# RegulatoryGenomicsGroup/chicdiff

Measured on AMD Instinct MI355X. Metric: interactions/sec NB-GLM Wald test, higher is better.
Workload: dtype f64; 1 GPU; synthetic 2000000 interactions x 8 samples (4v4), size factors + offsets(theta=0.5) + dispersions + Wald, design ~condition; rows_per_gpu=2000000, samples=8, global_rows=2000000, parallelism=rows-sharded x1, collectives=none (single rank), ranks_in_communicator=1

## Files before the change

### chicdiff_amd/csrc/api.hip

```cpp
#include <math.h>
#include <stdarg.h>
#include <stdio.h>
#include <stdlib.h>
#include <string.h>

#include <algorithm>
#include <mutex>
#include <thread>
#include <string>
#include <vector>
#include <unordered_set>

#include <dlfcn.h>

#include "common.h"
#include "prior_mc.h"

using namespace cd;

namespace cd {
struct ChinputCols {
    std::vector<int32_t> bait, oe, N;
    std::string error;
};
// ... 45 lines not shown
    struct EarlyCopy {
        int n = 0;
        struct Item { int col; char *pin; size_t bytes; } item[10];
        hipEvent_t ready = nullptr, done = nullptr;
        bool issued = false;
    } *early = nullptr;
    hipStream_t copy_stream = nullptr;
    hipEvent_t ev_fork = nullptr, ev_join = nullptr;
    std::vector<chicdiff_hip_ctx *> lanes;
    int cu_count = 0;
    hipStream_t own_stream = nullptr, stream = nullptr;
    chicdiff_allreduce_fn allreduce = nullptr;
    void *allreduce_user = nullptr;
    chicdiff_allgather_fn allgather = nullptr;
    void *allgather_user = nullptr;
    int world = 1, rank = 0;
    void *rccl_lib = nullptr, *rccl_comm = nullptr;
    int (*rccl_allreduce)(const void *, void *, size_t, int, int, void *, hipStream_t) = nullptr;
    int (*rccl_allgather)(const void *, void *, size_t, int, void *, hipStream_t) = nullptr;
    int (*rccl_comm_destroy)(void *) = nullptr;
    const char *(*rccl_error_string)(int) = nullptr;
    char err[512] = {0};
    int64_t cap_n = 0;
    int cap_S = 0;
    void *ws = nullptr;
    size_t ws_bytes = 0;
    char *aux = nullptr;
    size_t aux_bytes = 0;
    FitWork w{};
    double *d_sf = nullptr;
    double *d_logfact = nullptr;
    PmcTable *d_pmc[4] = {nullptr, nullptr, nullptr, nullptr};
    double *d_nf_tmp = nullptr;
    FitScalars *h_sc = nullptr;
    double *h_sf = nullptr;
    int timing = 0;
    std::vector<KTimer> timers;
    std::vector<std::pair<int, hipEvent_t>> pending;
    std::vector<hipEvent_t> event_pool;
    int scope_depth = 0;
    std::unordered_set<void *> user_allocs;
    std::mutex user_mu;
};

static char g_create_err[512];
constexpr int64_t kFuseOffsetsMaxRows = 1 << 18;

static const PmcTable &pmc_table(int df) {
    static PmcTable tables[4];
    static bool ready[4] = {false, false, false, false};
    static std::mutex mu;
    std::lock_guard<std::mutex> lock(mu);
    if (!ready[df]) {
        pmc_build(df, tables[df]);
        ready[df] = true;
    }
    return tables[df];
}

static int fail(chicdiff_hip_ctx *c, int code, const char *fmt, ...) {
    va_list ap;
    va_start(ap, fmt);
    vsnprintf(c ? c->err : g_create_err, 512, fmt, ap);
    va_end(ap);
    return code;
}
// ... 302 lines not shown
extern "C" int32_t chicdiff_hip_kernel_times(chicdiff_hip_ctx *c, chicdiff_kernel_time *out, int32_t cap) {
    if (!c) return 0;
    int32_t k = 0;
    for (auto &t : c->timers) {
        if (t.launches == 0) continue;
        if (out && k < cap) {
            out[k].name = t.name.c_str();
            out[k].ms = t.ms;
            out[k].launches = t.launches;
            out[k].bytes = t.bytes;
        }
        k++;
    }
    return k;
}

static size_t align256(size_t x) { return (x + 255) & ~(size_t)255; }

static int ensure_workspace(chicdiff_hip_ctx *c, int64_t n, int S) {
    if (c->ws && n <= c->cap_n && S <= c->cap_S) return CHICDIFF_OK;
    if (c->ws) {
        HIPCHK(c, hipStreamSynchronize(c->stream));
        HIPCHK(c, hipFree(c->ws));
        c->ws = nullptr;
    }
    const size_t nd = align256(sizeof(double) * (size_t)n), ni = align256(sizeof(int32_t) * (size_t)n);
    const size_t n_double_arrays = 15, n_int_arrays = 9;
    const size_t partials = align256(sizeof(double) * ((size_t)kRedBlocks * 72 + 128));
    const size_t hist = align256(sizeof(double) * (size_t)kMaxS * 2 * kSelBins);
    const size_t nfbytes = align256(sizeof(double) * (size_t)n * S);
    const size_t selcnt = align256(sizeof(double) * (size_t)kSelMaxWorld * kMaxS * 2);
    const size_t rowpack = align256((size_t)row_stride(S) * (size_t)n);
    const size_t start4 = align256(sizeof(double) * 4 * (size_t)n);
    const size_t total = nd * n_double_arrays + ni * n_int_arrays + partials + 2 * hist + selcnt + align256(sizeof(FitScalars)) + kQueueBytes + 1024 + kPlaceWords * 8 + nfbytes + rowpack + start4;
    hipError_t e = hipMalloc(&c->ws, total);
    if (e != hipSuccess) return fail(c, CHICDIFF_E_NOMEM, "workspace of %zu bytes: %s", total, hipGetErrorString(e));
    c->ws_bytes = total;
    char *p = (char *)c->ws;
    auto takeD = [&](double *&ptr) { ptr = (double *)p; p += nd; };
    auto takeI = [&](int32_t *&ptr) { ptr = (int32_t *)p; p += ni; };
    FitWork &w = c->w;
    takeD(w.baseMean); takeD(w.baseVar); takeD(w.gm0); takeD(w.gm1); takeD(w.rough); takeD(w.binit0); takeD(w.binit1);
    takeD(w.crow); takeD(w.dispGene); takeD(w.dispFit); takeD(w.dispMAP); takeD(w.disp); takeD(w.beta0); takeD(w.beta1);
    takeD(w.resid);
    takeI(w.allZero); takeI(w.geneIter); takeI(w.mapIter); takeI(w.outlier); takeI(w.betaIter); takeI(w.optimConv);
    takeI(w.order);
    { int32_t *q; takeI(q); w.cls = (uint8_t *)q; }
    takeI(w.gridlist);
    w.partials = (double *)p; p += partials;
    w.hist = (double *)p; p += hist;
    w.hist_local = (double *)p; p += hist;
    w.selcnt = (double *)p; p += selcnt;
    w.sc = (FitScalars *)p; p += align256(sizeof(FitScalars));
    w.logfact = c->d_logfact;
    w.queue = (unsigned long long *)p; p += kQueueBytes;
    w.barrier = (unsigned int *)p; p += 1024;
    w.place = (unsigned long long *)p; p += kPlaceWords * 8;
    c->d_nf_tmp = (double *)p; p += nfbytes;
    w.rowpack = p; p += rowpack;
    w.start = (double *)p;
    c->cap_n = n;
    c->cap_S = S;
    HIPCHK(c, hipMemsetAsync(w.sc, 0, align256(sizeof(FitScalars)) + kQueueBytes + 1024, c->stream));
    return CHICDIFF_OK;
}

static int ensure_aux(chicdiff_hip_ctx *c, size_t bytes) {
    if (c->aux_bytes >= bytes) return CHICDIFF_OK;
    if (c->aux) {
        HIPCHK(c, hipStreamSynchronize(c->stream));
        HIPCHK(c, hipFree(c->aux));
        c->aux = nullptr;
        c->aux_bytes = 0;
    }
    hipError_t e = hipMalloc((void **)&c->aux, bytes);
    if (e != hipSuccess) return fail(c, CHICDIFF_E_NOMEM, "scratch of %zu bytes: %s", bytes, hipGetErrorString(e));
    c->aux_bytes = bytes;
    return CHICDIFF_OK;
}

struct CollTimer {
    chicdiff_hip_ctx *c;
    int idx = -1;
    hipEvent_t e0 = nullptr, e1 = nullptr;
    CollTimer(chicdiff_hip_ctx *c_, const char *name, double bytes) : c(c_) {
        if (c->timing != 1) return;
        for (size_t i = 0; i < c->timers.size(); i++)
            if (c->timers[i].name == name) idx = (int)i;
        if (idx < 0) {
            KTimer t;
            t.name = name;
            c->timers.push_back(t);
            idx = (int)c->timers.size() - 1;
// ... 747 lines not shown
    auto cleanup = [&]() {
        if (early.issued) (void)hipStreamSynchronize(c->copy_stream);
        if (early.ready) (void)hipEventDestroy(early.ready);
        if (early.done) (void)hipEventDestroy(early.done);
    };
    if (rc) { cleanup(); return rc; }
    for (auto &q : cols) {
        if (q.early) continue;
        if (e == hipSuccess) e = hipEventCreateWithFlags(&q.ev, hipEventDisableTiming);
        if (e == hipSuccess) e = hipMemcpyAsync(q.pin, q.dev, q.bytes, hipMemcpyDeviceToHost, c->stream);
        if (e == hipSuccess) e = hipEventRecord(q.ev, c->stream);
    }
    if (e == hipSuccess && !cols.empty()) {
        std::sort(cols.begin(), cols.end(), [](const Col &x, const Col &y) { return x.early > y.early; });
        int nt = c->host.host_copy_threads < (int)cols.size() ? c->host.host_copy_threads : (int)cols.size();
        std::vector<std::thread> th;
        for (int t = 0; t < nt; t++)
            th.emplace_back([&, t]() {
                for (size_t k = t; k < cols.size(); k += nt) {
                    if (hipEventSynchronize(cols[k].early ? early.done : cols[k].ev) != hipSuccess) { trc[0] = 1; continue; }
                    memcpy(cols[k].host, cols[k].pin, cols[k].bytes);
                }
            });
        for (auto &w : th) w.join();
    }
    for (auto &q : cols) if (q.ev) (void)hipEventDestroy(q.ev);
    cleanup();
    if (e != hipSuccess || trc[0]) return fail(c, CHICDIFF_E_HIP, "D2H copy: %s", e != hipSuccess ? hipGetErrorString(e) : "event wait failed");
    return CHICDIFF_OK;
}

static int size_factors_impl(chicdiff_hip_ctx *c, const int32_t *d_counts, int64_t n, int32_t S, bool all_rounds) {
    Scope t(c, "size_factors");
    launch_row_ratio(d_counts, n, S, c->d_nf_tmp, c->d_carry, c->stream);
    SelArgs sa{};
    sa.mode = SEL_SIZEFACTOR;
    sa.ncol = S;
    sa.n = n;
    sa.ratio = c->d_nf_tmp;
    sa.S = S;
    sa.sf_out = c->d_sf;
    sa.overflow_out = c->d_carry;
    const int rc = run_select(c, sa, all_rounds);
    if (rc) return rc;
    if (c->host.fault_inject & 4) {
        c->host.fault_inject &= ~4;
        launch_poke(c->d_carry, 1, c->stream);
    }
    return CHICDIFF_OK;
}

static int sf_overflow_consensus(chicdiff_hip_ctx *c, bool *overflow) {
    double *d_flag = c->d_sf + kMaxS;
    launch_flag_to_double(c->d_carry, d_flag, c->stream);
    int rc = do_allreduce(c, d_flag, 1);
    if (rc) return rc;
    double h = 0;
    HIPCHK(c, hipMemcpyAsync(&h, d_flag, sizeof h, hipMemcpyDeviceToHost, c->stream));
    HIPCHK(c, hipStreamSynchronize(c->stream));
    *overflow = h > 0;
    return CHICDIFF_OK;
}

int chicdiff_hip_size_factors_dev(chicdiff_hip_ctx *c, const int32_t *d_counts, int64_t n, int32_t S, double *sf_host) {
    if (!c) return CHICDIFF_E_INVALID;
    int rc = (!d_counts || !sf_host || n < 1 || S < 1 || S > kMaxS) ? fail(c, CHICDIFF_E_INVALID, "size_factors: bad arguments") : CHICDIFF_OK;
    if ((rc = begin_call(c, rc, n, S))) return rc;
    bool all_rounds = c->host.select_all_rounds != 0, overflow = false;
    for (;;) {
        if ((rc = size_factors_impl(c, d_counts, n, S, all_rounds)) || (rc = sf_overflow_consensus(c, &overflow))) break;
        if (!overflow || all_rounds) break;
        all_rounds = true;
        c->refits++;
    }
    if (!rc) rc = read_scalars(c);
    timing_collect(c);
    if (rc) return rc;
// ... 220 lines not shown
    if (!d_counts || !d_nf || !d_log_alpha || !d_lp || !d_dlp || !d_alpha || !d_mu || K < 1 || live_rows < 0 || live_rows > 64 ||
        (d_prior_mean && !(prior_var > 0)))
        return fail(c, CHICDIFF_E_INVALID, "selftest_objective: bad arguments");
    if (int rc = check_counts_group(c, n, S, group, d)) return rc;
    if (int rc = check_opts(c, opts)) return rc;
    HIPCHK(c, hipSetDevice(c->device));
    if (int rc = ensure_workspace(c, n, S)) return rc;
    const Opts o = make_opts(c, opts, S);
    HIPCHK(c, hipMemsetAsync(c->w.sc, 0, align256(sizeof(FitScalars)) + kQueueBytes + 1024, c->stream));
    launch_prep(d_counts, const_cast<double *>(d_nf), d, c->w, o, c->stream);
    ObjectiveProbe pb{d_log_alpha, K, d_prior_mean, d_prior_mean ? 1.0 / prior_var : 0.0, live_rows, d_lp, d_dlp, d_alpha, d_mu};
    const int lanes = launch_objective_probe(d, c->w, o, pb, c->stream);
    HIPCHK(c, hipStreamSynchronize(c->stream));
    if (lanes < 0) return fail(c, CHICDIFF_E_INVALID, "selftest_objective: the line search has no samples-across-lanes layout for %d live rows at S = %d", live_rows, S);
    HIPCHK(c, hipGetLastError());
    if (lanes_per_row) *lanes_per_row = lanes;
    return CHICDIFF_OK;
}

extern "C" int chicdiff_hip_selftest_r_random(int32_t kind, uint32_t seed, double a, double b, int64_t n, double *out) {
    if (!out || n < 0 || kind < 0 || kind > 3) return CHICDIFF_E_INVALID;
    if (kind == 3 && !(a > 0 && b > 0)) return CHICDIFF_E_INVALID;
    RStream r(seed);
    for (int64_t i = 0; i < n; i++) out[i] = kind == 0 ? r.unif() : kind == 1 ? r.norm() : kind == 2 ? r.expo() : r.gamma(a, b);
    return CHICDIFF_OK;
}
extern "C" int chicdiff_hip_selftest_sched_class(int32_t mode, double min_disp, const double *alpha_init, const double *group_mean, int64_t n,
                                                 int32_t *cls_out, int32_t *bounds) {
    if (n < 0 || (n > 0 && (!alpha_init || !group_mean || !cls_out)) || mode < 1 || mode > 4) return CHICDIFF_E_INVALID;
    for (int64_t i = 0; i < n; i++) cls_out[i] = cd::sched_class(alpha_init[i], group_mean[i], min_disp, mode);
    if (bounds) for (int a = 0; a <= 6; a++) bounds[a] = cd::sched_classes_a(a, mode);
    return CHICDIFF_OK;
}
extern "C" int chicdiff_hip_selftest_queue_claim(uint64_t old, int32_t back, uint32_t chunks, uint32_t first_back, int32_t stop_percent, int32_t claimed,
                                                 uint32_t *chunk_out, int32_t *again_out) {
    uint32_t chunk = 0;
    const bool valid = cd::queue_claim(old, back != 0, chunks, chunk);
    if (chunk_out) *chunk_out = chunk;
    if (again_out) *again_out = cd::filler_claims(claimed != 0, old, chunks, first_back, cd::filler_stop_f(stop_percent, chunks, first_back));
    return valid ? 1 : 0;
}
extern "C" int chicdiff_hip_selftest_prior_mc(int32_t df, const double *hist40, double *dens_out, double *prior_var_out) {
    if (df < 1 || df > 3) return CHICDIFF_E_INVALID;
    const PmcTable &t = pmc_table(df);
    if (dens_out) memcpy(dens_out, t.dens, sizeof t.dens);
    if (prior_var_out) {
        if (!hist40) return CHICDIFF_E_INVALID;
        *prior_var_out = pmc_prior_var(hist40, t);
    }
    return CHICDIFF_OK;
}

extern "C" int chicdiff_hip_fragment_background_dev(chicdiff_hip_ctx *c, const int32_t *d_bait, const int32_t *d_oe, int64_t nru,
                                                    int32_t id_min, int32_t nid, const int64_t *d_midsum, int32_t S,
                                                    const double *d_sj, const double *d_si, const int32_t *d_tblb,
                                                    const int32_t *d_tlb, const double *d_T, int32_t ntblb, int32_t ntlb,
                                                    const double *distfun_host, double *d_bmean, double *d_tmean,
                                                    double *d_fullmean) {
    if (!c) return CHICDIFF_E_INVALID;
    if (!d_bait || !d_oe || !d_midsum || !d_sj || !d_si || !d_tblb || !d_tlb || !d_T || !distfun_host || nru < 0 || nid < 1 ||
        S < 1 || S > kMaxS || ntblb < 1 || ntlb < 1)
        return fail(c, CHICDIFF_E_INVALID, "fragment_background: bad arguments");
    HIPCHK(c, hipSetDevice(c->device));
    int rc = ensure_aux(c, sizeof(double) * 10 * kMaxS);
    if (rc) return rc;
    double *d_df = reinterpret_cast<double *>(c->aux);
// ... 389 lines not shown
```

### chicdiff_amd/csrc/common.h

```cpp
#pragma once
#include <hip/hip_runtime.h>
#include <stdint.h>

#include "../../include/chicdiff_hip.h"
#include "fit_driver.h"
#include "fit_state.h"

namespace cd {

constexpr int kRedBlocks = 1024;

struct FitDims {
    int64_t n;
    int32_t S, p, nA, nB;
    uint64_t gmask;
};

struct FitWork {
    double *baseMean, *baseVar, *gm0, *gm1, *rough, *binit0, *binit1, *crow;
    double *dispGene, *dispFit, *dispMAP, *disp, *beta0, *beta1, *resid;
    int32_t *allZero, *geneIter, *mapIter, *outlier, *betaIter, *optimConv;
    int32_t *order;
    uint8_t *cls;
    int32_t *gridlist;
// ... 143 lines not shown
void launch_dispfit_resid(FitDims d, FitWork w, Opts o, hipStream_t st);
void launch_prior_var(FitDims d, FitWork w, Opts o, hipStream_t st);
void launch_resid_hist(FitDims d, FitWork w, double *out40, hipStream_t st);
void launch_prior_mc(FitDims d, FitWork w, const double *hist40, const void *table, hipStream_t st);
void launch_wald_prep(const int32_t *counts, const double *nf, FitDims d, FitWork w, Opts o, hipStream_t st);
void launch_wald_irls(const int32_t *counts, const double *nf, FitDims d, FitWork w, Opts o, hipStream_t st);
void launch_wald_final(const int32_t *counts, const double *nf, FitDims d, FitWork w, Opts o,
                       const chicdiff_nbglm_out &out, hipStream_t st);
void launch_wald_intercept(const int32_t *counts, const double *nf, FitDims d, FitWork w, Opts o,
                           const chicdiff_nbglm_out &out, hipStream_t st);
void launch_dev_sum_finish(FitDims d, FitWork w, const int32_t *carry, const double *sf_dev, hipStream_t st);

struct SelArgs {
    int mode;
    int ncol;
    int64_t n;
    const double *resid;
    const double *ratio;
    int S;
    int shift;
    double *sf_out;
    int32_t *overflow_out;
};
void launch_sel_hist(SelArgs a, FitWork w, hipStream_t st);
void launch_sel_step(SelArgs a, FitWork w, hipStream_t st);
void launch_sel_shortcut(SelArgs a, FitWork w, hipStream_t st);
void launch_sel_finish(SelArgs a, FitWork w, hipStream_t st);
void launch_sel_keep_local(SelArgs a, FitWork w, hipStream_t st);
void launch_sel_gather_counts(SelArgs a, FitWork w, int world, int rank, hipStream_t st);
void launch_sel_gather_place(SelArgs a, FitWork w, int world, int rank, hipStream_t st);
void launch_sel_gather_finish(SelArgs a, FitWork w, int world, int rank, hipStream_t st);

void launch_row_ratio(const int32_t *counts, int64_t n, int S, double *ratio, int32_t *clear_flag, hipStream_t st);
void launch_offsets(const double *fullMean, const double *sf_dev, int64_t n, int S, double theta, int mix,
                    double *out, hipStream_t st);
void launch_window_sums(const int32_t *fragN, const double *fragFM, int64_t nfrag, int S, const int64_t *rptr,
                        int64_t n, int32_t *N, double *FM, hipStream_t st);
size_t count_join_scratch_bytes(int64_t nkeys);
void launch_count_join(const int32_t *bait, const int32_t *oe, int64_t nru, const int64_t *keys,
                       const int32_t *vals, int64_t nkeys, int32_t *out, void *scratch, hipStream_t st);
void launch_fragment_background(const int32_t *bait, const int32_t *oe, int64_t nru, int32_t id_min, int32_t nid,
                                const int64_t *midsum, int32_t S, const double *sj, const double *si, const int32_t *tblb,
                                const int32_t *tlb, const double *T, int32_t ntblb, int32_t ntlb, const double *distfun_dev,
                                double *bmean, double *tmean, double *fullmean, hipStream_t st);
size_t bh_workspace_bytes(int64_t n);
int launch_bh_adjust(const double *p, int64_t n, double *padj, char *ws, hipStream_t st);
size_t ihw_workspace_bytes();
void launch_ihw_apply(const double *avDist, const double *pvalue, int64_t n, const double *breaks, const double *weights,
                      int ng, int32_t *group, double *weight, double *wp, double *partials, hipStream_t st);
void launch_cooks_filter(const int32_t *counts, int64_t n, int S, int p, const double *maxCooks, const int32_t *argmax,
                         double cutoff, double *pvalue, unsigned long long *nout, hipStream_t st);
size_t if_workspace_bytes(int64_t n);
int run_independent_filtering(const double *d_bm, const double *d_p, int64_t n, double alpha, double *d_padj, char *ws, hipStream_t st,
                              hipStream_t st2, hipEvent_t fork, hipEvent_t join, chicdiff_results_info *info);
size_t ct_workspace_bytes(int64_t n);
int launch_count_table(const int32_t *bait, const int32_t *oe, const int32_t *N, int64_t n, const uint8_t *keep, int32_t max_id,
                       int64_t *keys_out, int32_t *vals_out, char *ws, hipStream_t st);
size_t ru_scan_bytes(int64_t n);
int launch_ru_count(const int32_t *bait, const int32_t *oe, int64_t n, int s, const int32_t *chr_of, int maxfrag,
                    int64_t *region_ptr, int32_t *minOE, int32_t *maxOE, int *bad, void *tmp, size_t tmp_bytes, hipStream_t st,
                    unsigned int *mask_out = nullptr);
void launch_ru_fill(const int32_t *bait, const int32_t *oe, int64_t n, int s, const int32_t *chr_of, int maxfrag,
                    const int64_t *region_ptr, int32_t *ru_bait, int32_t *ru_region, int32_t *ru_oe, hipStream_t st,
                    const unsigned int *mask_in = nullptr);
void launch_region_avdist(const int32_t *bait, const int32_t *oe, const int64_t *ptr, int64_t n, int32_t id_min, int32_t nid,
                          const int64_t *midsum, const int32_t *chr, double *avDist, hipStream_t st);
// ... 26 lines not shown
```

### chicdiff_amd/csrc/global_kernels.hip

```cpp
#include "common.h"
#include "devmath.h"
#include "prior_mc.h"

namespace cd {

template <int K>
__device__ __forceinline__ void block_reduce_store(double (&v)[K], double *out) {
    __shared__ double red[K][4];
    const int lane = threadIdx.x & 63, wave = threadIdx.x >> 6;
#pragma unroll
    for (int k = 0; k < K; k++) {
        double x = v[k];
        for (int off = 32; off > 0; off >>= 1) x += __shfl_down(x, off);
        if (lane == 0) red[k][wave] = x;
    }
    __syncthreads();
    if (threadIdx.x < K) out[threadIdx.x] = (red[threadIdx.x][0] + red[threadIdx.x][1]) + (red[threadIdx.x][2] + red[threadIdx.x][3]);
}

__global__ void reduce_partials_kernel(const double *partials, int nblk, int K, double *sums) {
    __shared__ double red[256];
    for (int k = 0; k < K; k++) {
        double acc = 0;
        for (int b = threadIdx.x; b < nblk; b += 256) acc += partials[(int64_t)b * K + k];
// ... 1086 lines not shown
    const int64_t step = (int64_t)gridDim.x * 256;
    int32_t kn[16];
    int64_t i = blockIdx.x * 256 + threadIdx.x;
#pragma unroll
    for (int j = 0; j < 16; j++) kn[j] = (j < S && i < n) ? counts[(int64_t)j * n + i] : 1;
    for (; i < n; i += step) {
        double l[16];
        int32_t kc[16];
#pragma unroll
        for (int j = 0; j < 16; j++) kc[j] = kn[j];
        if (i + step < n) {
#pragma unroll
            for (int j = 0; j < 16; j++) kn[j] = j < S ? counts[(int64_t)j * n + i + step] : 1;
        }
#pragma unroll
        for (int j = 0; j < 16; j++) {
            const int32_t k = kc[j];
            l[j] = k > 0 ? tlog((double)k, s_lt) : (k == 0 ? -INFINITY : NAN);
        }
        double s = 0;
#pragma unroll
        for (int j = 0; j < 16; j++)
            if (j < S) s += l[j];
        const double lg = s / S;
        const bool use = isfinite(lg);
#pragma unroll
        for (int j = 0; j < 16; j++)
            if (j < S) ratio[(int64_t)j * n + i] = use ? l[j] - lg : NAN;
    }
}
void launch_row_ratio(const int32_t *counts, int64_t n, int S, double *ratio, int32_t *clear_flag, hipStream_t st) {
    if (S <= 16) row_ratio16_kernel<<<kRedBlocks * 2, 256, 0, st>>>(counts, n, S, ratio, clear_flag);
    else row_ratio_kernel<<<kRedBlocks, 256, 0, st>>>(counts, n, S, ratio, clear_flag);
}

__device__ __forceinline__ double rlog(double x) { return (x > 0.0 && x < 1.7e308) ? flog(x) : log(x); }

__global__ __launch_bounds__(256) void offsets16_kernel(const double *__restrict__ fm, const double *__restrict__ sf,
                                                        int64_t n, int S, double theta, int mix,
                                                        double *__restrict__ out) {
    __shared__ LogEntry s_lt[64];
    log_table_to_lds(s_lt);
    for (int64_t i = blockIdx.x * 256 + threadIdx.x; i < n; i += (int64_t)gridDim.x * 256) {
        double v[16];
#pragma unroll
        for (int j = 0; j < 16; j++) v[j] = j < S ? fm[(int64_t)j * n + i] : 1.0;
        offsets_row16(v, S, sf, theta, mix, s_lt);
#pragma unroll
        for (int j = 0; j < 16; j++)
            if (j < S) out[(int64_t)j * n + i] = v[j];
    }
}

__global__ __launch_bounds__(256) void offsets_kernel(const double *__restrict__ fm, const double *__restrict__ sf,
                                                      int64_t n, int S, double theta, int mix,
                                                      double *__restrict__ out) {
    for (int64_t i = blockIdx.x * 256 + threadIdx.x; i < n; i += (int64_t)gridDim.x * 256) {
        double sl = 0;
        for (int j = 0; j < S; j++) sl += rlog(fm[(int64_t)j * n + i]);
        const double gmean = exp(sl / S);
        bool anyna = false;
        for (int j = 0; j < S; j++) {
            const double m3 = fm[(int64_t)j * n + i] / gmean;
            anyna |= (m3 != m3);
        }
        double g2 = 1.0;
// ... 746 lines not shown
```

### chicdiff_amd/hip.py

```python
from __future__ import annotations

import ctypes as C
import os

import numpy as np

from .dist import ALLGATHER_FN, ALLREDUCE_FN

_HERE = os.path.dirname(os.path.abspath(__file__))
LIB_PATH = os.path.join(_HERE, "lib", "libchicdiff_hip.so")

ST_TREND_FAILED, ST_PRIORVAR_MC, ST_BETA_NONCONV, ST_ALLZERO_ROWS, ST_TREND_LOCAL = 1, 2, 4, 8, 16


EXPORTS = [
    "chicdiff_hip_create", "chicdiff_hip_destroy", "chicdiff_hip_last_error", "chicdiff_hip_set_stream",
    "chicdiff_hip_set_allreduce", "chicdiff_hip_set_allgather", "chicdiff_hip_last_refits", "chicdiff_hip_set_option", "chicdiff_hip_default_opts", "chicdiff_hip_size_factors_dev",
    "chicdiff_hip_offsets_dev", "chicdiff_hip_window_sums_dev", "chicdiff_hip_count_join_dev",
    "chicdiff_hip_fragment_background_dev", "chicdiff_hip_bh_adjust_dev", "chicdiff_hip_ihw_apply_dev",
    "chicdiff_hip_region_universe_count_dev", "chicdiff_hip_region_universe_fill_dev", "chicdiff_hip_region_universe_dev", "chicdiff_hip_count_table_dev",
    "chicdiff_hip_chinput_read", "chicdiff_hip_chinput_table_dev", "chicdiff_hip_region_avdist_dev",
    "chicdiff_hip_count_join_inner_dev", "chicdiff_hip_count_join_multi_dev", "chicdiff_hip_region_assemble_dev",
    "chicdiff_hip_malloc", "chicdiff_hip_free", "chicdiff_hip_outstanding_allocations", "chicdiff_hip_memcpy_h2d", "chicdiff_hip_memcpy_d2h",
    "chicdiff_hip_rccl_unique_id", "chicdiff_hip_rccl_init", "chicdiff_hip_cooks_filter_dev",
    "chicdiff_hip_independent_filtering_dev",
    "chicdiff_hip_nbglm_fit_dev", "chicdiff_hip_nbglm_fit", "chicdiff_hip_wald_test_dev", "chicdiff_hip_theta_grid_dev",
    "chicdiff_hip_wald_pvalues_dev", "chicdiff_hip_selftest_math_dev", "chicdiff_hip_selftest_math3_dev", "chicdiff_hip_selftest_objective_dev", "chicdiff_hip_selftest_r_random", "chicdiff_hip_selftest_sched_class", "chicdiff_hip_selftest_queue_claim",
    "chicdiff_hip_selftest_prior_mc", "chicdiff_hip_selftest_chinput", "chicdiff_hip_kernel_times", "chicdiff_hip_enable_timing",
]


class Opts(C.Structure):
    _fields_ = [("minDisp", C.c_double), ("dispTol", C.c_double), ("kappa0", C.c_double),
                ("maxit", C.c_int32), ("betaMaxit", C.c_int32), ("betaTol", C.c_double),
                ("minmu", C.c_double), ("outlierSD", C.c_double), ("dispPriorVar", C.c_double),
                ("trendCoef", C.c_double * 2), ("fitType", C.c_int32), ("_pad", C.c_int32)]


OUT_DOUBLE = ["baseMean", "baseVar", "dispGeneEst", "dispFit", "dispMAP", "dispersion", "log2FoldChange",
              "lfcSE", "stat", "pvalue", "intercept", "interceptSE", "deviance", "maxCooks"]
OUT_INT = ["dispGeneIter", "dispIter", "dispOutlier", "betaConv", "betaIter", "allZero", "cooksArgmax"]


class Out(C.Structure):
    _fields_ = [(k, C.c_void_p) for k in OUT_DOUBLE + OUT_INT]


class Scalars(C.Structure):
    _fields_ = [("trendCoef", C.c_double * 2), ("varLogDispEsts", C.c_double), ("dispPriorVar", C.c_double),
                ("sumDeviance", C.c_double), ("nAllZero", C.c_int64), ("trendOuterIter", C.c_int32),
                ("status", C.c_int32)]


class ResultsInfo(C.Structure):
    _fields_ = [("filterThreshold", C.c_double), ("filterTheta", C.c_double), ("alpha", C.c_double), ("index", C.c_int32),
                ("_pad", C.c_int32), ("theta", C.c_double * 50), ("numRej", C.c_double * 50), ("lowess", C.c_double * 50)]


class KernelTime(C.Structure):
    _fields_ = [("name", C.c_char_p), ("ms", C.c_double), ("launches", C.c_int32), ("_pad", C.c_int32), ("bytes", C.c_double)]
# ... 525 lines not shown
```

### include/chicdiff_hip.h

```cpp
#ifndef CHICDIFF_HIP_H
#define CHICDIFF_HIP_H

#include <stdint.h>

#ifdef __cplusplus
extern "C" {
#endif

#define CHICDIFF_OK 0
#define CHICDIFF_E_INVALID 1
#define CHICDIFF_E_HIP 2
#define CHICDIFF_E_NOMEM 3
#define CHICDIFF_E_COMM 4
#define CHICDIFF_E_NUMERIC 5

#define CHICDIFF_ST_TREND_FAILED 1
#define CHICDIFF_ST_PRIORVAR_MC 2
#define CHICDIFF_ST_BETA_NONCONV 4
#define CHICDIFF_ST_ALLZERO_ROWS 8
#define CHICDIFF_ST_TREND_LOCAL 16

typedef struct chicdiff_hip_ctx chicdiff_hip_ctx;

typedef int (*chicdiff_allreduce_fn)(void *user, void *dev_buf, int64_t count);
// ... 151 lines not shown
                               int32_t S, const int32_t *group, const chicdiff_nbglm_opts *opts,
                               const chicdiff_nbglm_out *d_out, chicdiff_nbglm_scalars *scalars);

int chicdiff_hip_nbglm_fit(chicdiff_hip_ctx *ctx, const int32_t *counts, const double *nf, int64_t n, int32_t S,
                           const int32_t *group, const chicdiff_nbglm_opts *opts, const chicdiff_nbglm_out *out,
                           chicdiff_nbglm_scalars *scalars);

int chicdiff_hip_wald_test_dev(chicdiff_hip_ctx *ctx, const int32_t *d_counts, const double *d_fullMean, int64_t n,
                               int32_t S, const int32_t *group, double theta, const chicdiff_nbglm_opts *opts,
                               const chicdiff_nbglm_out *d_out, chicdiff_nbglm_scalars *scalars, double *sf_host);

int chicdiff_hip_theta_grid_dev(chicdiff_hip_ctx *ctx, const int32_t *d_counts, const double *d_fullMean,
                                const double *sf_host, int64_t n, int32_t S, const double *thetas,
                                int32_t ntheta, const chicdiff_nbglm_opts *opts, double *deviances_host);

int chicdiff_hip_wald_pvalues_dev(chicdiff_hip_ctx *ctx, const double *d_stat, int64_t n, double *d_p);

int chicdiff_hip_selftest_math_dev(chicdiff_hip_ctx *ctx, int32_t op, const double *d_x, int64_t n, double *d_out);
int chicdiff_hip_selftest_math3_dev(chicdiff_hip_ctx *ctx, int32_t op, const double *d_x, const double *d_y, int64_t n, double *d_out,
                                    double *d_out2);
int chicdiff_hip_selftest_objective_dev(chicdiff_hip_ctx *ctx, const int32_t *d_counts, const double *d_nf, int64_t n, int32_t S,
                                        const int32_t *group, const chicdiff_nbglm_opts *opts, const double *d_log_alpha, int32_t K,
                                        const double *d_prior_mean, double prior_var, int32_t live_rows, double *d_lp, double *d_dlp,
                                        double *d_alpha, double *d_mu, int32_t *lanes_per_row);

int chicdiff_hip_selftest_chinput(const char *path, int32_t nthreads, int64_t cap, int32_t *bait, int32_t *oe, int32_t *N,
                                  int64_t *nrows, char *err, int32_t errcap);
int chicdiff_hip_selftest_r_random(int32_t kind, uint32_t seed, double a, double b, int64_t n, double *out);
int chicdiff_hip_selftest_prior_mc(int32_t df, const double *hist40, double *dens_out, double *prior_var_out);
int chicdiff_hip_selftest_sched_class(int32_t mode, double min_disp, const double *alpha_init, const double *group_mean, int64_t n,
                                      int32_t *cls_out, int32_t *bounds);
int chicdiff_hip_selftest_queue_claim(uint64_t old, int32_t back, uint32_t chunks, uint32_t first_back, int32_t stop_percent, int32_t claimed,
                                      uint32_t *chunk_out, int32_t *again_out);

typedef struct {
    const char *name;
    double ms;
    int32_t launches;
    int32_t _pad;
    double bytes;
} chicdiff_kernel_time;
int32_t chicdiff_hip_kernel_times(chicdiff_hip_ctx *ctx, chicdiff_kernel_time *out, int32_t cap);
int chicdiff_hip_enable_timing(chicdiff_hip_ctx *ctx, int32_t on);

#ifdef __cplusplus
}
#endif
#endif
```

Baseline: 570.9 million interactions/s.

## Compute size-factor medians via binned histogram selection instead of radix select

For single-rank runs with up to 16 samples, the size-factor median of log-ratios is now found directly from counts. A histogram pass over fixed-width bins locates the median bin per column, a second pass collects candidates in those bins, and a finish kernel resolves the exact value with a sub-bin histogram and rank counting (or a radix fallback). This replaces the row_ratio pass that materialised the n×S ratio array and the multi-round radix select. It adds four new kernels and LDS-heavy atomics. Correctness depends on bin-range clamping and on the fallback paths for skewed distributions.

```diff
diff --git a/chicdiff_amd/csrc/api.hip b/chicdiff_amd/csrc/api.hip
--- a/chicdiff_amd/csrc/api.hip
+++ b/chicdiff_amd/csrc/api.hip
@@ -101,6 +101,8 @@
     double *d_logfact = nullptr;
     PmcTable *d_pmc[4] = {nullptr, nullptr, nullptr, nullptr};
     double *d_nf_tmp = nullptr;
+    unsigned int *d_sfhist = nullptr;
+    bool sfhist_dirty = false;
     FitScalars *h_sc = nullptr;
     double *h_sf = nullptr;
     int timing = 0;
@@ -469,7 +471,7 @@
     const size_t selcnt = align256(sizeof(double) * (size_t)kSelMaxWorld * kMaxS * 2);
     const size_t rowpack = align256((size_t)row_stride(S) * (size_t)n);
     const size_t start4 = align256(sizeof(double) * 4 * (size_t)n);
-    const size_t total = nd * n_double_arrays + ni * n_int_arrays + partials + 2 * hist + selcnt + align256(sizeof(FitScalars)) + kQueueBytes + 1024 + kPlaceWords * 8 + nfbytes + rowpack + start4;
+    const size_t total = nd * n_double_arrays + ni * n_int_arrays + partials + 2 * hist + selcnt + align256(sizeof(FitScalars)) + kQueueBytes + 1024 + kPlaceWords * 8 + nfbytes + rowpack + start4 + align256(sizeof(unsigned int) * kSfWorkWords);
     hipError_t e = hipMalloc(&c->ws, total);
     if (e != hipSuccess) return fail(c, CHICDIFF_E_NOMEM, "workspace of %zu bytes: %s", total, hipGetErrorString(e));
     c->ws_bytes = total;
@@ -495,7 +497,9 @@
     w.place = (unsigned long long *)p; p += kPlaceWords * 8;
     c->d_nf_tmp = (double *)p; p += nfbytes;
     w.rowpack = p; p += rowpack;
-    w.start = (double *)p;
+    w.start = (double *)p; p += start4;
+    c->d_sfhist = (unsigned int *)p;
+    c->sfhist_dirty = true;
     c->cap_n = n;
     c->cap_S = S;
     HIPCHK(c, hipMemsetAsync(w.sc, 0, align256(sizeof(FitScalars)) + kQueueBytes + 1024, c->stream));
@@ -1309,7 +1313,6 @@
 
 static int size_factors_impl(chicdiff_hip_ctx *c, const int32_t *d_counts, int64_t n, int32_t S, bool all_rounds) {
     Scope t(c, "size_factors");
-    launch_row_ratio(d_counts, n, S, c->d_nf_tmp, c->d_carry, c->stream);
     SelArgs sa{};
     sa.mode = SEL_SIZEFACTOR;
     sa.ncol = S;
@@ -1318,8 +1321,18 @@
     sa.S = S;
     sa.sf_out = c->d_sf;
     sa.overflow_out = c->d_carry;
-    const int rc = run_select(c, sa, all_rounds);
-    if (rc) return rc;
+    if (S <= kSfMaxS && !c->allreduce && !all_rounds) {
+        if (c->sfhist_dirty) HIPCHK(c, hipMemsetAsync(c->d_sfhist, 0, sizeof(unsigned int) * kSfWorkWords, c->stream));
+        c->sfhist_dirty = true;
+        launch_sf_direct(d_counts, n, S, sa, c->w, c->d_sfhist, reinterpret_cast<uint64_t *>(c->d_nf_tmp), c->d_carry,
+                         c->cu_count, c->stream);
+        HIPCHK(c, hipGetLastError());
+        c->sfhist_dirty = false;
+    } else {
+        launch_row_ratio(d_counts, n, S, c->d_nf_tmp, c->d_carry, c->stream);
+        const int rc = run_select(c, sa, all_rounds);
+        if (rc) return rc;
+    }
     if (c->host.fault_inject & 4) {
         c->host.fault_inject &= ~4;
         launch_poke(c->d_carry, 1, c->stream);
@@ -1606,6 +1619,17 @@
     if (bounds) for (int a = 0; a <= 6; a++) bounds[a] = cd::sched_classes_a(a, mode);
     return CHICDIFF_OK;
 }
+extern "C" int chicdiff_hip_selftest_sf_bin(int32_t S, const double *x, int64_t n, int32_t *nbins_out, int32_t *bin_out, int32_t sub_of,
+                                            int32_t *sub_out) {
+    if (S < 1 || S > cd::kSfMaxS || n < 0 || (n > 0 && (!x || !bin_out))) return CHICDIFF_E_INVALID;
+    const int nb = cd::sf_bins(S);
+    if (nbins_out) *nbins_out = nb;
+    for (int64_t i = 0; i < n; i++) {
+        bin_out[i] = cd::sf_bin(x[i], nb);
+        if (sub_out) sub_out[i] = cd::sf_sub_bin(x[i], nb, sub_of);
+    }
+    return CHICDIFF_OK;
+}
 extern "C" int chicdiff_hip_selftest_queue_claim(uint64_t old, int32_t back, uint32_t chunks, uint32_t first_back, int32_t stop_percent, int32_t claimed,
                                                  uint32_t *chunk_out, int32_t *again_out) {
     uint32_t chunk = 0;
diff --git a/chicdiff_amd/csrc/common.h b/chicdiff_amd/csrc/common.h
--- a/chicdiff_amd/csrc/common.h
+++ b/chicdiff_amd/csrc/common.h
@@ -199,6 +199,24 @@
 void launch_sel_gather_finish(SelArgs a, FitWork w, int world, int rank, hipStream_t st);
 
 void launch_row_ratio(const int32_t *counts, int64_t n, int S, double *ratio, int32_t *clear_flag, hipStream_t st);
+
+constexpr double kSfBinLo = -4.0, kSfBinSpan = 8.0;
+constexpr int kSfHistWords = 15360;
+constexpr int kSfSubBins = 4096;
+constexpr int kSfMaxS = 16;
+constexpr int kSfWorkWords = kSfHistWords + 2 * kSfMaxS * 32;
+__host__ __device__ inline int sf_bins(int S) { return kSfHistWords / (S <= 4 ? 4 : S <= 8 ? 8 : 16); }
+__host__ __device__ inline double sf_bin_pos(double x, int nb) { return (x - kSfBinLo) * ((double)nb / kSfBinSpan); }
+__host__ __device__ inline int sf_bin(double x, int nb) {
+    const double u = floor(sf_bin_pos(x, nb));
+    return u < 0.0 ? 0 : (u > (double)(nb - 1) ? nb - 1 : (int)u);
+}
+__host__ __device__ inline int sf_sub_bin(double x, int nb, int b) {
+    const double u = floor((sf_bin_pos(x, nb) - (double)b) * (double)kSfSubBins);
+    return u < 0.0 ? 0 : (u > (double)(kSfSubBins - 1) ? kSfSubBins - 1 : (int)u);
+}
+void launch_sf_direct(const int32_t *counts, int64_t n, int S, SelArgs a, FitWork w, unsigned int *hist, uint64_t *lists,
+                      int32_t *clear_flag, int cus, hipStream_t st);
 void launch_offsets(const double *fullMean, const double *sf_dev, int64_t n, int S, double theta, int mix,
                     double *out, hipStream_t st);
 void launch_window_sums(const int32_t *fragN, const double *fragFM, int64_t nfrag, int S, const int64_t *rptr,
diff --git a/chicdiff_amd/csrc/global_kernels.hip b/chicdiff_amd/csrc/global_kernels.hip
--- a/chicdiff_amd/csrc/global_kernels.hip
+++ b/chicdiff_amd/csrc/global_kernels.hip
@@ -1142,6 +1142,362 @@
 void launch_row_ratio(const int32_t *counts, int64_t n, int S, double *ratio, int32_t *clear_flag, hipStream_t st) {
     if (S <= 16) row_ratio16_kernel<<<kRedBlocks * 2, 256, 0, st>>>(counts, n, S, ratio, clear_flag);
     else row_ratio_kernel<<<kRedBlocks, 256, 0, st>>>(counts, n, S, ratio, clear_flag);
+}
+
+
+template <int SM>
+__device__ __forceinline__ bool sf_row_keys(const int32_t (&kc)[SM], int S, const LogEntry *lt, double (&x)[SM]) {
+    double l[SM];
+#pragma unroll
+    for (int j = 0; j < SM; j++) {
+        const int32_t k = kc[j];
+        l[j] = k > 0 ? tlog((double)k, lt) : (k == 0 ? -INFINITY : NAN);
+    }
+    double s = 0;
+#pragma unroll
+    for (int j = 0; j < SM; j++)
+        if (j < S) s += l[j];
+    const double lg = s / S;
+#pragma unroll
+    for (int j = 0; j < SM; j++) x[j] = l[j] - lg;
+    return isfinite(lg);
+}
+
+__device__ __forceinline__ void sf_hist_add(unsigned int *h, bool valid, unsigned int bin) {
+    unsigned long long todo = __ballot(valid);
+    const int lane = threadIdx.x & 63;
+    for (int it = 0; it < 4 && todo; it++) {
+        const int leader = __ffsll((long long)todo) - 1;
+        const unsigned int bl = (unsigned int)__builtin_amdgcn_readlane((int)bin, leader);
+        const unsigned long long same = __ballot(valid && bin == bl) & todo;
+        const int cnt = __popcll(same);
+        if (lane == leader) atomicAdd(&h[bl], (unsigned int)cnt);
+        todo &= ~same;
+        if (cnt < 4) break;
+    }
+    if ((todo >> lane) & 1ull) atomicAdd(&h[bin], 1u);
+}
+
+constexpr int kSfThreads = 1024;
+constexpr int kSfStage = 4096;
+constexpr int kSfCntStride = 32;
+
+__device__ __forceinline__ void sf_wg_pick(const unsigned int *h, int nb, int nr, bool from_total, double (&rank)[2], int (&bin)[2],
+                                           double (&rin)[2], unsigned int (&cnt)[2], double &total_out) {
+    __shared__ double sh_scan[kSfThreads / 64], sh_rin[2];
+    __shared__ int sh_bin[2];
+    __shared__ unsigned int sh_cnt[2];
+    const int tid = threadIdx.x, lane = tid & 63, wave = tid >> 6;
+    const int per = (nb + kSfThreads - 1) / kSfThreads;
+    double mine[4] = {0, 0, 0, 0}, acc = 0;
+#pragma unroll
+    for (int q = 0; q < 4; q++) {
+        const int b = tid * per + q;
+        if (q < per && b < nb) mine[q] = (double)h[b];
+        acc += mine[q];
+    }
+    double incl = acc;
+    for (int off = 1; off < 64; off <<= 1) {
+        const double o = __shfl_up(incl, off);
+        if (lane >= off) incl += o;
+    }
+    if (lane == 63) sh_scan[wave] = incl;
+    __syncthreads();
+    double before_wave = 0, total = 0;
+    for (int q = 0; q < kSfThreads / 64; q++) {
+        if (q < wave) before_wave += sh_scan[q];
+        total += sh_scan[q];
+    }
+    incl += before_wave;
+    const double before = incl - acc;
+    const bool last_thread = tid == (nb - 1) / per;
+    if (from_total) {
+        const int64_t mi = (int64_t)total;
+        rank[0] = (double)((mi - 1) / 2);
+        rank[1] = (double)(mi / 2);
+    }
+    for (int s = 0; s < nr; s++) {
+        const double r = rank[s];
+        if ((before <= r && r < incl) || (last_thread && r >= incl && incl == total)) {
+            double cum = before;
+            int q = 0;
+            for (; q < per - 1 && tid * per + q < nb - 1; q++) {
+                if (cum + mine[q] > r) break;
+                cum += mine[q];
+            }
+            sh_bin[s] = tid * per + q;
+            sh_rin[s] = r - cum;
+            sh_cnt[s] = (unsigned int)mine[q];
+        }
+    }
+    __syncthreads();
+    for (int s = 0; s < nr; s++) {
+        bin[s] = sh_bin[s];
+        rin[s] = sh_rin[s];
+        cnt[s] = sh_cnt[s];
+    }
+    total_out = total;
+    __syncthreads();
+}
+
+template <int SM>
+__global__ __launch_bounds__(kSfThreads) void sf_hist_kernel(const int32_t *__restrict__ counts, int64_t n, int S, int nb,
+                                                            unsigned int *__restrict__ ghist, int32_t *clear_flag) {
+    if (clear_flag && blockIdx.x == 0 && threadIdx.x == 0) *clear_flag = 0;
+    __shared__ LogEntry s_lt[64];
+    __shared__ unsigned int s_h[kSfHistWords];
+    const int words = S * nb;
+    for (int k = threadIdx.x; k < words; k += kSfThreads) s_h[k] = 0;
+    log_table_to_lds(s_lt);
+    const int64_t step = (int64_t)gridDim.x * kSfThreads;
+    int32_t kn[SM];
+    int64_t i = (int64_t)blockIdx.x * kSfThreads + threadIdx.x;
+#pragma unroll
+    for (int j = 0; j < SM; j++) kn[j] = (j < S && i < n) ? counts[(int64_t)j * n + i] : 1;
+    for (; i < n; i += step) {
+        int32_t kc[SM];
+        double x[SM];
+#pragma unroll
+        for (int j = 0; j < SM; j++) kc[j] = kn[j];
+        if (i + step < n) {
+#pragma unroll
+            for (int j = 0; j < SM; j++) kn[j] = j < S ? counts[(int64_t)j * n + i + step] : 1;
+        }
+        const bool use = sf_row_keys<SM>(kc, S, s_lt, x);
+#pragma unroll
+        for (int j = 0; j < SM; j++)
+            if (j < S) sf_hist_add(s_h + j * nb, use, (unsigned int)sf_bin(x[j], nb));
+    }
+    __syncthreads();
+    for (int k = threadIdx.x; k < words; k += kSfThreads) {
+        const unsigned int c = s_h[k];
+        if (c) atomicAdd(&ghist[k], c);
+    }
+}
+
+__global__ __launch_bounds__(kSfThreads) void sf_pick_kernel(FitWork w, unsigned int *ghist, unsigned int *gcnt, int nb) {
+    const int col = blockIdx.x;
+    FitScalars *sc = w.sc;
+    unsigned int *g = ghist + (size_t)col * nb;
+    double rank[2], rin[2], total;
+    int bin[2];
+    unsigned int cnt[2];
+    sf_wg_pick(g, nb, 2, true, rank, bin, rin, cnt, total);
+    for (int k = threadIdx.x; k < nb; k += kSfThreads) g[k] = 0;
+    if (threadIdx.x < 2) {
+        const int slot = threadIdx.x;
+        sc->sel_prefix[2 * col + slot] = (uint64_t)(total > 0 ? bin[slot] : nb);
+        sc->sel_rank[2 * col + slot] = rin[slot];
+        gcnt[(2 * col + slot) * kSfCntStride] = 0;
+        if (slot == 0) sc->sel_count[col] = total;
+        if (slot == 0 && col == 0) sc->sel_fast_done = 0;
+    }
+}
+
+template <int SM>
+__global__ __launch_bounds__(kSfThreads) void sf_list_kernel(const int32_t *__restrict__ counts, int64_t n, int S, int nb, FitWork w,
+                                                            unsigned int *__restrict__ gcnt, uint64_t *__restrict__ lists) {
+    __shared__ LogEntry s_lt[64];
+    __shared__ int s_b[2][kSfMaxS];
+    __shared__ uint64_t s_key[kSfStage];
+    __shared__ unsigned char s_tag[kSfStage];
+    __shared__ unsigned int s_n, s_lc[2 * kSfMaxS], s_base[2 * kSfMaxS];
+    const FitScalars *sc = w.sc;
+    if ((int)threadIdx.x < 2 * S) s_b[threadIdx.x & 1][threadIdx.x >> 1] = (int)sc->sel_prefix[threadIdx.x];
+    if (threadIdx.x < 2 * kSfMaxS) s_lc[threadIdx.x] = 0;
+    if (threadIdx.x == 0) s_n = 0;
+    log_table_to_lds(s_lt);
+    const int lane = threadIdx.x & 63;
+    const int64_t step = (int64_t)gridDim.x * kSfThreads;
+    int32_t kn[SM];
+    int64_t i = (int64_t)blockIdx.x * kSfThreads + threadIdx.x;
+#pragma unroll
+    for (int j = 0; j < SM; j++) kn[j] = (j < S && i < n) ? counts[(int64_t)j * n + i] : 1;
+    for (; i < n; i += step) {
+        int32_t kc[SM];
+        double x[SM];
+#pragma unroll
+        for (int j = 0; j < SM; j++) kc[j] = kn[j];
+        if (i + step < n) {
+#pragma unroll
+            for (int j = 0; j < SM; j++) kn[j] = j < S ? counts[(int64_t)j * n + i + step] : 1;
+        }
+        const bool use = sf_row_keys<SM>(kc, S, s_lt, x);
+        unsigned int hit = 0;
+#pragma unroll
+        for (int j = 0; j < SM; j++)
+            if (j < S) {
+                const int b = sf_bin(x[j], nb);
+                const int b0 = s_b[0][j], b1 = s_b[1][j];
+                hit |= (b == b0 ? 1u : 0u) << j;
+                hit |= (b != b0 && b == b1 ? 1u : 0u) << (16 + j);
+            }
+        if (!use) hit = 0;
+        unsigned int over = 0;
+        if (hit != 0) {
+#pragma unroll
+            for (int j = 0; j < SM; j++)
+#pragma unroll
+                for (int slot = 0; slot < 2; slot++)
+                    if (j < S && ((hit >> (16 * slot + j)) & 1u)) {
+                        const unsigned int pos = atomicAdd(&s_n, 1u);
+                        if (pos < (unsigned int)kSfStage) {
+                            s_key[pos] = key_of(x[j]);
+                            s_tag[pos] = (unsigned char)(2 * j + slot);
+                        } else over |= 1u << (16 * slot + j);
+                    }
+        }
+        if (__ballot(over != 0) == 0ull) continue;
+#pragma unroll
+        for (int j = 0; j < SM; j++)
+            if (j < S) {
+#pragma unroll
+                for (int slot = 0; slot < 2; slot++) {
+                    const bool m = (over >> (16 * slot + j)) & 1u;
+                    const unsigned long long mask = __ballot(m);
+                    if (mask == 0ull) continue;
+                    const int leader = __ffsll((long long)mask) - 1;
+                    unsigned int base = 0;
+                    if (lane == leader) base = atomicAdd(&gcnt[(2 * j + slot) * kSfCntStride], (unsigned int)__popcll(mask));
+                    base = (unsigned int)__shfl((int)base, leader);
+                    if (m) {
+                        const int64_t pos = (int64_t)base + __popcll(mask & ((1ull << lane) - 1ull));
+                        lists[(int64_t)j * n + (slot ? n - 1 - pos : pos)] = key_of(x[j]);
+                    }
+                }
+            }
+    }
+    __syncthreads();
+    const int staged = (int)(s_n < (unsigned int)kSfStage ? s_n : (unsigned int)kSfStage);
+    for (int e = threadIdx.x; e < staged; e += kSfThreads) atomicAdd(&s_lc[s_tag[e]], 1u);
+    __syncthreads();
+    if ((int)threadIdx.x < 2 * S) {
+        const unsigned int c = s_lc[threadIdx.x];
+        s_base[threadIdx.x] = c ? atomicAdd(&gcnt[threadIdx.x * kSfCntStride], c) : 0u;
+        s_lc[threadIdx.x] = 0;
+    }
+    __syncthreads();
+    for (int e = threadIdx.x; e < staged; e += kSfThreads) {
+        const int t = s_tag[e], j = t >> 1;
+        const int64_t pos = (int64_t)s_base[t] + atomicAdd(&s_lc[t], 1u);
+        lists[(int64_t)j * n + ((t & 1) ? n - 1 - pos : pos)] = s_key[e];
+    }
+}
+
+constexpr int kSfCand = 1024;
+__device__ __forceinline__ uint64_t sf_list_at(const uint64_t *list, int64_t n, bool back, int64_t e) { return list[back ? n - 1 - e : e]; }
+
+__device__ __forceinline__ void sf_list_select(const uint64_t *list, int64_t n, bool back, int64_t m, int nb, int b, int nr,
+                                               double (&rk)[2], unsigned int *s_h, uint64_t *s_c, unsigned int *s_nc, uint64_t *s_res) {
+    const int tid = threadIdx.x;
+    for (int k = tid; k < kSfSubBins; k += kSfThreads) s_h[k] = 0;
+    __syncthreads();
+    for (int64_t e = tid; e < m; e += kSfThreads)
+        sf_hist_add(s_h, true, (unsigned int)sf_sub_bin(value_of(sf_list_at(list, n, back, e)), nb, b));
+    __syncthreads();
+    int sb[2];
+    double rin[2], total;
+    unsigned int cnt[2];
+    sf_wg_pick(s_h, kSfSubBins, nr, false, rk, sb, rin, cnt, total);
+    for (int q = 0; q < nr; q++) {
+        const bool shared = nr == 2 && sb[0] == sb[1] && cnt[0] <= (unsigned int)kSfCand;
+        if (q == 1 && shared) break;
+        if (cnt[q] <= (unsigned int)kSfCand) {
+            if (tid == 0) *s_nc = 0;
+            __syncthreads();
+            for (int64_t e = tid; e < m; e += kSfThreads) {
+                const uint64_t key = sf_list_at(list, n, back, e);
+                if (sf_sub_bin(value_of(key), nb, b) == sb[q]) s_c[atomicAdd(s_nc, 1u)] = key;
+            }
+            __syncthreads();
+            const int nc = (int)cnt[q];
+            if (tid < nc) {
+                const uint64_t mine = s_c[tid];
+                int less = 0;
+                for (int k = 0; k < nc; k++) {
+                    const uint64_t o = s_c[k];
+                    less += (o < mine || (o == mine && k < tid)) ? 1 : 0;
+                }
+                if ((double)less == rin[q]) s_res[q] = mine;
+                if (shared && (double)less == rin[1]) s_res[1] = mine;
+            }
+            __syncthreads();
+        } else {
+            uint64_t p = 0;
+            double r[2] = {rk[q], 0};
+            for (int round = 0; round < 6; round++) {
+                const int shift = kSelShifts[round], bits = sel_bits(shift), hi = shift + bits;
+                const uint64_t dmask = (1ull << bits) - 1ull;
+                for (int k = tid; k < kSelBins; k += kSfThreads) s_h[k] = 0;
+                __syncthreads();
+                for (int64_t e = tid; e < m; e += kSfThreads) {
+                    const uint64_t key = sf_list_at(list, n, back, e);
+                    sf_hist_add(s_h, sel_match(key, p, hi), (unsigned int)((key >> shift) & dmask));
+                }
+                __syncthreads();
+                int rb[2];
+                double rr[2], rt;
+                unsigned int rc[2];
+                sf_wg_pick(s_h, 1 << bits, 1, false, r, rb, rr, rc, rt);
+                p |= (uint64_t)rb[0] << shift;
+                r[0] = rr[0];
+            }
+            if (tid == 0) s_res[q] = p;
+            __syncthreads();
+        }
+    }
+}
+
+__global__ __launch_bounds__(kSfThreads) void sf_finish_kernel(SelArgs a, FitWork w, int nb, const unsigned int *__restrict__ gcnt,
+                                                              const uint64_t *__restrict__ lists) {
+    __shared__ unsigned int s_h[kSelBins > kSfSubBins ? kSelBins : kSfSubBins];
+    __shared__ uint64_t s_c[kSfCand], s_res[2];
+    __shared__ unsigned int s_nc;
+    const int col = blockIdx.x;
+    FitScalars *sc = w.sc;
+    const int b0 = (int)sc->sel_prefix[2 * col], b1 = (int)sc->sel_prefix[2 * col + 1];
+    const double rank0 = sc->sel_rank[2 * col], rank1 = sc->sel_rank[2 * col + 1];
+    const int64_t m0 = gcnt[2 * col * kSfCntStride], m1 = gcnt[(2 * col + 1) * kSfCntStride];
+    const bool empty = !(sc->sel_count[col] > 0);
+    const uint64_t *list = lists + (int64_t)col * a.n;
+    if (threadIdx.x < 2) s_res[threadIdx.x] = 0xFFFFFF0000000000ull;
+    __syncthreads();
+    if (!empty) {
+        if (b0 == b1) {
+            double rk[2] = {rank0, rank1};
+            const int nr = rank0 == rank1 ? 1 : 2;
+            sf_list_select(list, a.n, false, m0, nb, b0, nr, rk, s_h, s_c, &s_nc, s_res);
+            if (nr == 1 && threadIdx.x == 0) s_res[1] = s_res[0];
+        } else {
+            double rk[2] = {rank0, 0};
+            sf_list_select(list, a.n, false, m0, nb, b0, 1, rk, s_h, s_c, &s_nc, s_res);
+            rk[0] = rank1;
+            sf_list_select(list, a.n, true, m1, nb, b1, 1, rk, s_h, s_c, &s_nc, s_res + 1);
+        }
+    }
+    __syncthreads();
+    if (threadIdx.x == 0) {
+        sc->sel_prefix[2 * col] = s_res[0];
+        sc->sel_prefix[2 * col + 1] = s_res[1];
+        if (col == 0) sc->sel_fast_done = 1;
+        sel_finish_col(a, sc, col);
+    }
+}
+
+void launch_sf_direct(const int32_t *counts, int64_t n, int S, SelArgs a, FitWork w, unsigned int *hist, uint64_t *lists,
+                      int32_t *clear_flag, int cus, hipStream_t st) {
+    const int nb = sf_bins(S);
+    int64_t hb = (n + kSfThreads - 1) / kSfThreads;
+    if (hb > (cus > 0 ? cus : 256)) hb = cus > 0 ? cus : 256;
+    unsigned int *gcnt = hist + kSfHistWords;
+    if (S <= 4) sf_hist_kernel<4><<<(unsigned)hb, kSfThreads, 0, st>>>(counts, n, S, nb, hist, clear_flag);
+    else if (S <= 8) sf_hist_kernel<8><<<(unsigned)hb, kSfThreads, 0, st>>>(counts, n, S, nb, hist, clear_flag);
+    else sf_hist_kernel<16><<<(unsigned)hb, kSfThreads, 0, st>>>(counts, n, S, nb, hist, clear_flag);
+    sf_pick_kernel<<<S, kSfThreads, 0, st>>>(w, hist, gcnt, nb);
+    if (S <= 4) sf_list_kernel<4><<<(unsigned)hb, kSfThreads, 0, st>>>(counts, n, S, nb, w, gcnt, lists);
+    else if (S <= 8) sf_list_kernel<8><<<(unsigned)hb, kSfThreads, 0, st>>>(counts, n, S, nb, w, gcnt, lists);
+    else sf_list_kernel<16><<<(unsigned)hb, kSfThreads, 0, st>>>(counts, n, S, nb, w, gcnt, lists);
+    sf_finish_kernel<<<S, kSfThreads, 0, st>>>(a, w, nb, gcnt, lists);
 }
 
 __device__ __forceinline__ double rlog(double x) { return (x > 0.0 && x < 1.7e308) ? flog(x) : log(x); }
diff --git a/chicdiff_amd/hip.py b/chicdiff_amd/hip.py
--- a/chicdiff_amd/hip.py
+++ b/chicdiff_amd/hip.py
@@ -25,7 +25,7 @@
     "chicdiff_hip_rccl_unique_id", "chicdiff_hip_rccl_init", "chicdiff_hip_cooks_filter_dev",
     "chicdiff_hip_independent_filtering_dev",
     "chicdiff_hip_nbglm_fit_dev", "chicdiff_hip_nbglm_fit", "chicdiff_hip_wald_test_dev", "chicdiff_hip_theta_grid_dev",
-    "chicdiff_hip_wald_pvalues_dev", "chicdiff_hip_selftest_math_dev", "chicdiff_hip_selftest_math3_dev", "chicdiff_hip_selftest_objective_dev", "chicdiff_hip_selftest_r_random", "chicdiff_hip_selftest_sched_class", "chicdiff_hip_selftest_queue_claim",
+    "chicdiff_hip_wald_pvalues_dev", "chicdiff_hip_selftest_math_dev", "chicdiff_hip_selftest_math3_dev", "chicdiff_hip_selftest_objective_dev", "chicdiff_hip_selftest_r_random", "chicdiff_hip_selftest_sched_class", "chicdiff_hip_selftest_queue_claim", "chicdiff_hip_selftest_sf_bin",
     "chicdiff_hip_selftest_prior_mc", "chicdiff_hip_selftest_chinput", "chicdiff_hip_kernel_times", "chicdiff_hip_enable_timing",
 ]
 
diff --git a/include/chicdiff_hip.h b/include/chicdiff_hip.h
--- a/include/chicdiff_hip.h
+++ b/include/chicdiff_hip.h
@@ -207,6 +207,7 @@
                                       int32_t *cls_out, int32_t *bounds);
 int chicdiff_hip_selftest_queue_claim(uint64_t old, int32_t back, uint32_t chunks, uint32_t first_back, int32_t stop_percent, int32_t claimed,
                                       uint32_t *chunk_out, int32_t *again_out);
+int chicdiff_hip_selftest_sf_bin(int32_t S, const double *x, int64_t n, int32_t *nbins_out, int32_t *bin_out, int32_t sub_of, int32_t *sub_out);
 
 typedef struct {
     const char *name;
```

Measured after the change: 583.2 million interactions/s (median of 6 runs). 2.2% higher.
